# cristianpjensen/thesis-pai-reconstruction

Hardware: AMD Instinct MI355X
Metric: train images/sec (256x256, bs=64) Pix2Pix step (higher is better)
Workload: dtype bf16; 1 GPU; Pix2Pix generator+PatchGAN GAN step, 256x256x1 pairs, 64 images/GPU (BASELINE configs[1]); global_batch=64, per_gpu_batch=64, loss_type=gan, parallelism=dp1, grad_bucket_dtype=f32

## Files before the change

thesis-pai-reconstruction_amd/csrc/gg_thin.hip:

```cpp
#include <stdlib.h>

#include "common.h"

#ifndef THIN_ABL
#define THIN_ABL 0
#endif
typedef __attribute__((ext_vector_type(8))) __bf16 bf8_t;
typedef __attribute__((ext_vector_type(4))) __bf16 bf4_t;
typedef __attribute__((ext_vector_type(4))) float f4_t;
typedef __attribute__((ext_vector_type(8))) short s8_t;
typedef __attribute__((ext_vector_type(8))) unsigned short us8_t;

__device__ uint4 g_zero_line_thin[16];


__device__ __forceinline__ bf8_t relu8(bf8_t f) {
    s8_t x = __builtin_bit_cast(s8_t, f);
    const s8_t z = {0, 0, 0, 0, 0, 0, 0, 0};
    return __builtin_bit_cast(bf8_t, __builtin_elementwise_max(x, z));
}

template <int S>
__device__ __forceinline__ us8_t thin_gather8(__amdgpu_buffer_rsrc_t rs, int e0, int ix0, int TW, bool valid) {
    typedef __attribute__((ext_vector_type(4))) unsigned u4_t;
    const int base = ix0 & ~1, o = ix0 & 1;
    const bool neg = valid && e0 + base < 0;
    const unsigned vo = valid ? (neg ? 0u : (unsigned)(e0 + base) * 2u) : 0x80000000u;
    unsigned out[4];
    if (S == 2) {
        u4_t a = __builtin_amdgcn_raw_buffer_load_b128(rs, (int)vo, 0, 0);
        u4_t b = __builtin_amdgcn_raw_buffer_load_b128(rs, (int)vo + 16, 0, 0);
        if (__builtin_amdgcn_ballot_w64(neg) != 0) {
            if (neg) { b = (u4_t){a[3], b[0], b[1], b[2]}; a = (u4_t){0u, a[0], a[1], a[2]}; }
        }
        const unsigned sel = o ? 0x07060302u : 0x05040100u;
        out[0] = __builtin_amdgcn_perm(a[1], a[0], sel);
        out[1] = __builtin_amdgcn_perm(a[3], a[2], sel);
        out[2] = __builtin_amdgcn_perm(b[1], b[0], sel);
        out[3] = __builtin_amdgcn_perm(b[3], b[2], sel);
    } else {
        u4_t a = __builtin_amdgcn_raw_buffer_load_b128(rs, (int)vo, 0, 0);
        unsigned a4 = __builtin_amdgcn_raw_buffer_load_b32(rs, (int)vo + 16, 0, 0);
        if (__builtin_amdgcn_ballot_w64(neg) != 0) {
            if (neg) { a4 = a[3]; a = (u4_t){0u, a[0], a[1], a[2]}; }
        }
        const unsigned sh = (unsigned)o * 16u;
        out[0] = __builtin_amdgcn_alignbit(a[1], a[0], sh);
        out[1] = __builtin_amdgcn_alignbit(a[2], a[1], sh);
        out[2] = __builtin_amdgcn_alignbit(a[3], a[2], sh);
        out[3] = __builtin_amdgcn_alignbit(a4, a[3], sh);
    }
    const bool edge = valid && (ix0 < 0 || ix0 + S * 7 >= TW);
    if (__builtin_amdgcn_ballot_w64(edge) != 0) {
#pragma unroll
        for (int i = 0; i < 4; ++i) {
            const bool lo = (unsigned)(ix0 + S * (2 * i)) < (unsigned)TW, hi = (unsigned)(ix0 + S * (2 * i + 1)) < (unsigned)TW;
            out[i] &= (lo ? 0xffffu : 0u) | (hi ? 0xffff0000u : 0u);
        }
    }
    us8_t r;
#pragma unroll
    for (int i = 0; i < 4; ++i) { r[2 * i] = (unsigned short)(out[i] & 0xffffu); r[2 * i + 1] = (unsigned short)(out[i] >> 16); }
    return r;
}

__device__ __forceinline__ unsigned relu2u(unsigned v) {
    typedef __attribute__((ext_vector_type(2))) short s2_t;
    const s2_t z = {0, 0};
    return __builtin_bit_cast(unsigned, __builtin_elementwise_max(__builtin_bit_cast(s2_t, v), z));
}

__device__ __forceinline__ uint2 thin_gather4(__amdgpu_buffer_rsrc_t rs, int e0, int ix0, int TW, bool valid) {
    typedef __attribute__((ext_vector_type(3))) unsigned u3_t;
    const int base = ix0 & ~1, o = ix0 & 1;
    const bool neg = valid && e0 + base < 0;
    const unsigned vo = valid ? (neg ? 0u : (unsigned)(e0 + base) * 2u) : 0x80000000u;
    u3_t a = __builtin_amdgcn_raw_buffer_load_b96(rs, (int)vo, 0, 0);
    if (__builtin_amdgcn_ballot_w64(neg) != 0) {
        if (neg) a = (u3_t){0u, a[0], a[1]};
    }
    const unsigned sh = (unsigned)o * 16u;
    uint2 out = make_uint2(__builtin_amdgcn_alignbit(a[1], a[0], sh), __builtin_amdgcn_alignbit(a[2], a[1], sh));
    const bool edge = valid && (ix0 < 0 || ix0 + 3 >= TW);
    if (__builtin_amdgcn_ballot_w64(edge) != 0) {
        out.x &= ((unsigned)ix0 < (unsigned)TW ? 0xffffu : 0u) | ((unsigned)(ix0 + 1) < (unsigned)TW ? 0xffff0000u : 0u);
        out.y &= ((unsigned)(ix0 + 2) < (unsigned)TW ? 0xffffu : 0u) | ((unsigned)(ix0 + 3) < (unsigned)TW ? 0xffff0000u : 0u);
    }
    return out;
}

__device__ __forceinline__ void decode_row2(const GG& g, int m, int& n, int& gy, int& gx) {
    if (g.lw >= 0) {
        gx = m & (g.OWg - 1);
        gy = (m >> g.lw) & (g.OHg - 1);
        n = m >> (g.lw + g.lh);
    } else {
        gx = m % g.OWg;
        int r = m / g.OWg;
        gy = r % g.OHg;
        n = r / g.OHg;
    }
}

bool thin_fwd_ok(int dtype, const GG& g, const FwdArgs& a) {
    const bool taps_ok = g.ntaps == 16 || (g.ntaps == 9 && g.S == 1 && g.C2 == 0);
    return dtype == PAI_BF16 && g.nphase == 1 && taps_ok && g.OS == 1 && g.C1 == 1 && g.C2 <= 1 &&
           (g.Cout % 64) == 0 && g.Cout <= 128 && !a.stats && !a.yf32 && !a.skip_d1 &&
           (g.D2 == 0 || (g.D1 % 16) == 0);
}

template <int T>
__global__ __launch_bounds__(256) void thin_fwd_k(GG g, FwdArgs a, int fast_ok) {
    const int tid = threadIdx.x, lane = tid & 63, wid = tid >> 6;
    const int fr = lane & 15, fq = lane >> 4;
    const bf16_t* x1 = (const bf16_t*)a.x1;
    const bf16_t* x2 = (const bf16_t*)a.x2;
    const bf16_t* w = (const bf16_t*)a.w;
    const int mtiles = g.Cout / 16;
    const int KT = g.ntaps * T;
    const bool sect = (fast_ok & 2) != 0;
    fast_ok &= 1;

    bf8_t af[8];
#pragma unroll
    for (int mt = 0; mt < 8; ++mt) {
        us8_t z = {0, 0, 0, 0, 0, 0, 0, 0};
        const int co = sect ? 64 * (mt >> 2) + 32 * ((mt & 3) >> 1) + 8 * (fr >> 2) + 4 * (mt & 1) + (fr & 3)
                            : 64 * (mt >> 2) + 16 * (fr >> 2) + 4 * (mt & 3) + (fr & 3);
        if (mt < mtiles) {
            if ((KT & 7) == 0) {
                if (8 * fq < KT) z = *(const us8_t*)(w + (size_t)co * KT + 8 * fq);
            } else {
#pragma unroll
                for (int e = 0; e < 8; ++e)
                    if (8 * fq + e < KT) z[e] = w[(size_t)co * KT + 8 * fq + e];
            }
        }
        af[mt] = __builtin_bit_cast(bf8_t, z);
    }
    float bias[2][16];
#pragma unroll
    for (int gq = 0; gq < 2; ++gq)
#pragma unroll
        for (int e = 0; e < 16; ++e)
            bias[gq][e] = (a.bias && gq * 4 < mtiles) ? a.bias[64 * gq + (sect ? 32 * (e >> 3) + 8 * fq + (e & 7) : 16 * fq + e)] : 0.f;
    int pdy[8], pdx[8];
// ... 597 lines not shown
        const int hy0 = (oyl >> 1) + 1, hx0 = (oxl >> 1) + 1;
        const size_t o = ((size_t)n * g.OH + oy) * g.OW + ox;
#pragma unroll
        for (int tt = 0; tt < T; ++tt) {
            const int t = t0 + tt;
            float v = a.bias ? a.bias[t] : 0.f;
#pragma unroll
            for (int k = 0; k < 4; ++k) {
                const int e = tab[ph][k];
                const int hy = hy0 + (int)(signed char)(e & 0xff), hx = hx0 + (int)(signed char)((e >> 8) & 0xff);
                v += Ys[tt][hy * TU_HW + hx][(e >> 16) & 0xff];
            }
            if (t < g.D1) {
                if (a.y1 && !a.skip_d1) ((bf16_t*)a.y1)[o * g.D1 + t] = f2bf(v);
            } else if (a.y2) {
                ((bf16_t*)a.y2)[o * g.D2 + (t - g.D1)] = f2bf(v);
            }
            if (a.yact || a.yf32) {
                const float av = act_apply(v, a.eact);
                if (a.yact) ((bf16_t*)a.yact)[o * g.Cout + t] = f2bf(av);
                if (a.yf32) a.yf32[o * g.Cout + t] = av;
            }
        }
    }
}

static bool thin_up_ok(const GG& g) {
    return pai_tunable("thin_up", 1) && g.nphase == 4 && g.ntaps == 4 && g.OS == 2 && g.wtaps == 16 && (g.H % 16) == 0 &&
           (g.W % 16) == 0 && (g.Cin == 64 || g.Cin == 128);
}

int launch_thin_dgrad(const GG& g, const FwdArgs& a, hipStream_t s) {
    const int T = thin_dgrad_T(g, a);
    const int t0 = (g.Cout == 2 && a.skip_d1) ? 1 : 0;
    if (thin_up_ok(g)) {
        const int tx = g.W / 16, ty = g.H / 16;
        const dim3 grid(g.N * tx * ty);
        if (T == 1 && g.Cin == 128) PAI_LAUNCH((thin_up_k<1, 4>), grid, dim3(256), 0, s, g, a, t0, tx, ty);
        else if (T == 1) PAI_LAUNCH((thin_up_k<1, 2>), grid, dim3(256), 0, s, g, a, t0, tx, ty);
        else if (g.Cin == 128) PAI_LAUNCH((thin_up_k<2, 4>), grid, dim3(256), 0, s, g, a, t0, tx, ty);
        else PAI_LAUNCH((thin_up_k<2, 2>), grid, dim3(256), 0, s, g, a, t0, tx, ty);
        PAI_LAUNCH_CHECK();
        return 0;
    }
    int blocks = cdiv((int64_t)g.N * g.H * g.W, 256);
    if (blocks > 4096) blocks = 4096;
#define TDG(TT, KK) PAI_LAUNCH((thin_dgrad_gemm_k<TT, KK>), dim3(blocks), dim3(256), 0, s, g, a, pai_ctx()->scratch, t0)
#define TDG_K(TT)                                     \
    switch (g.Cin / 32) {                             \
        case 1: TDG(TT, 1); break;                    \
        case 2: TDG(TT, 2); break;                    \
        case 4: TDG(TT, 4); break;                    \
        case 8: TDG(TT, 8); break;                    \
        case 16: TDG(TT, 16); break;                  \
        default: PAI_CHECK(false, "thin dgrad: unsupported Cin %d", g.Cin); \
    }
    if (T == 1) { TDG_K(1) } else { TDG_K(2) }
#undef TDG_K
#undef TDG
    PAI_LAUNCH_CHECK();
    PAI_CHECK((int64_t)g.N * g.OH * g.OW < (1ll << 31), "thin dgrad: more than 2^31 output pixels");
    int64_t b2 = ((int64_t)g.N * g.OH * g.OW + 255) / 256;
    if (b2 > 8192) b2 = 8192;
    PAI_LAUNCH(thin_col2im_k, dim3((int)b2), dim3(256), 0, s, g, a, (const float*)pai_ctx()->scratch, T, t0);
    PAI_LAUNCH_CHECK();
    return 0;
}

struct ThinW {
    const bf16_t *thin1, *thin2;
    const bf16_t *wide1, *wide2;
    int N, H, W, TH, TW, WC1, WC2;
    int relu1, relu2;
    int lw, lh;
    int tmul, flip;
    int kw, ntaps;
    float* dw;
    int s_wc, s_tap, s_t;
    float* dbias;
    int M;
    int fast;
    int pair;
    float* partial;
};

__device__ __forceinline__ int tw_swz(int row) { return ((row & 3) << 2) | ((row >> 2) & 3); }
__device__ __forceinline__ unsigned tw_off(int row, int ch) { return (unsigned)(256 * row + 16 * (ch ^ tw_swz(row))); }

#ifndef THIN_WG_WAVES
#define THIN_WG_WAVES 1
#endif
template <int T>
__global__ __launch_bounds__(256, THIN_WG_WAVES) void thin_wgrad_k(ThinW p, int chunks_per_block) {
    extern __shared__ __attribute__((aligned(16))) unsigned char smem[];
    const int tid = threadIdx.x, lane = tid & 63;
    const int wid = __builtin_amdgcn_readfirstlane(tid >> 6);
    const int fr = lane & 15, fq = lane >> 4, tq = fr >> 2, tp = fr & 3;
    const int wc0 = blockIdx.y * 128;
    const int WC = min(p.WC1 + p.WC2 - wc0, 128);
    const int pair = p.pair;
    const int ntile = pair ? 8 : WC / 16;
    const int ks = wid & 1;
    const int nt0 = (wid >> 1) * (ntile / 2);
    const int ntn = ntile / 2;
    const int pixh = pair ? (wid >> 1) * 64 : 0;
    const int CH = pair ? 128 : 64;
    const bf16_t* zero = (const bf16_t*)g_zero_line_thin;

    const int sc = lane & 15, sr = wid * 4 + (lane >> 4);
    const int gch = sc ^ tw_swz(sr);
    const bf16_t* wsrc;
    int wstride, wcol;
    bool wvalid = pair || gch * 8 < WC;
    const int wpix = pair ? (gch >> 3) * 64 : 0;
    if (pair) { wsrc = p.wide1; wstride = p.WC1; wcol = (gch & 7) * 8; }
    else if (wc0 + gch * 8 < p.WC1) { wsrc = p.wide1; wstride = p.WC1; wcol = wc0 + gch * 8; }
    else { wsrc = p.wide2; wstride = p.WC2; wcol = gch * 8 - p.WC1; }

    int kdy[T], kdx[T];
    const bf16_t* ksrc[T];
    int kt[T];
#pragma unroll
    for (int tt = 0; tt < T; ++tt) {
        const int k = 16 * tt + fr;
        const int tap = k / T, t = k - tap * T;
        const int th = tap / p.kw, tw = tap - th * p.kw;
        kdy[tt] = p.flip ? 1 - th : th - 1;
        kdx[tt] = tap < p.ntaps ? (p.flip ? 1 - tw : tw - 1) : -(1 << 20);
        ksrc[tt] = t ? p.thin2 : p.thin1;
        kt[tt] = t;
    }
    const unsigned thin_bytes = (unsigned)(p.N * p.TH * p.TW) * 2u;
    const __amdgpu_buffer_rsrc_t trs1 = __builtin_amdgcn_make_buffer_rsrc(const_cast<bf16_t*>(p.thin1), 0, thin_bytes, 0x00020000);
    const __amdgpu_buffer_rsrc_t trs2 = __builtin_amdgcn_make_buffer_rsrc(
        const_cast<bf16_t*>(p.thin2 ? p.thin2 : p.thin1), 0, p.thin2 ? thin_bytes : 0u, 0x00020000);

    f4_t acc[T][4];
#pragma unroll
    for (int tt = 0; tt < T; ++tt)
#pragma unroll
        for (int j = 0; j < 4; ++j) acc[tt][j] = (f4_t){0.f, 0.f, 0.f, 0.f};
    f4_t accb[4];
#pragma unroll
    for (int j = 0; j < 4; ++j) accb[j] = (f4_t){0.f, 0.f, 0.f, 0.f};
    const unsigned one2 = fr == 0 ? 0x3f803f80u : 0u;
    const bf8_t ones = __builtin_bit_cast(bf8_t, make_uint4(one2, one2, one2, one2));

    for (int ci = 0; ci < chunks_per_block; ++ci) {
        const int p0 = (blockIdx.x * chunks_per_block + ci) * CH;
        if (p0 >= p.M) break;
#pragma unroll
        for (int j = 0; j < 4; ++j) {
            const int m = p0 + wpix + sr + 16 * j;
            const bf16_t* src = (wvalid && m < p.M) ? wsrc + (size_t)m * wstride + wcol : zero;
            __builtin_amdgcn_global_load_lds((const __attribute__((address_space(1))) void*)src,
                                             (__attribute__((address_space(3))) void*)(smem + (16 * j + wid * 4) * 256),
                                             16, 0, 0);
        }
        bf8_t af[T];
#pragma unroll
        for (int tt = 0; tt < T; ++tt) {
            us8_t pv;
            if (p.fast) {
                const int m = p0 + pixh + 32 * ks + 8 * fq;
                int n, ay, bx;
                if (p.lw >= 0) { bx = m & (p.W - 1); ay = (m >> p.lw) & (p.H - 1); n = m >> (p.lw + p.lh); }
                else { bx = m % p.W; const int r = m / p.W; ay = r % p.H; n = r / p.H; }
                const int iy = p.tmul * ay + kdy[tt], ix0 = p.tmul * bx + kdx[tt];
                const bool rowok = m < p.M && (unsigned)iy < (unsigned)p.TH && kdx[tt] > -(1 << 19);
                const int e0 = (n * p.TH + iy) * p.TW;
                if (p.tmul == 2) pv = kt[tt] ? thin_gather8<2>(trs2, e0, ix0, p.TW, rowok) : thin_gather8<2>(trs1, e0, ix0, p.TW, rowok);
                else pv = kt[tt] ? thin_gather8<1>(trs2, e0, ix0, p.TW, rowok) : thin_gather8<1>(trs1, e0, ix0, p.TW, rowok);
            } else {
#pragma unroll
            for (int j = 0; j < 8; ++j) {
                const int m = p0 + pixh + 32 * ks + 8 * fq + j;
                int n, ay, bx;
                if (p.lw >= 0) { bx = m & (p.W - 1); ay = (m >> p.lw) & (p.H - 1); n = m >> (p.lw + p.lh); }
                else { bx = m % p.W; const int r = m / p.W; ay = r % p.H; n = r / p.H; }
                const int iy = p.tmul * ay + kdy[tt], ix = p.tmul * bx + kdx[tt];
                const bool inb = m < p.M && (unsigned)iy < (unsigned)p.TH && (unsigned)ix < (unsigned)p.TW;
                pv[j] = inb ? ksrc[tt][(size_t)(n * p.TH + iy) * p.TW + ix] : (unsigned short)0;
            }
            }
            af[tt] = __builtin_bit_cast(bf8_t, pv);
        }
        __syncthreads();
#pragma unroll
        for (int nt = 0; nt < 4; ++nt) {
            if (nt >= ntn) break;
            const int col0 = (nt0 + nt) * 16;
            bf8_t bfr;
#pragma unroll
            for (int h = 0; h < 2; ++h) {
                const int row = ks * 32 + fq * 8 + h * 4 + tq;
                const int ch = col0 / 8 + (tp >> 1);
                bf4_t v = __builtin_amdgcn_ds_read_tr16_b64_v4bf16(
                    (bf4_t __attribute__((address_space(3)))*)(smem + tw_off(row, ch) + 8 * (tp & 1)));
#pragma unroll
                for (int e = 0; e < 4; ++e) bfr[h * 4 + e] = v[e];
            }
            if ((pair || wc0 + col0 < p.WC1) ? p.relu1 : p.relu2) bfr = relu8(bfr);
#pragma unroll
            for (int tt = 0; tt < T; ++tt)
                acc[tt][nt] = __builtin_amdgcn_mfma_f32_16x16x32_bf16(af[tt], bfr, acc[tt][nt], 0, 0, 0);
            if (p.dbias) accb[nt] = __builtin_amdgcn_mfma_f32_16x16x32_bf16(ones, bfr, accb[nt], 0, 0, 0);
        }
        __syncthreads();
    }
    float* part0 = p.partial ? p.partial + (((size_t)blockIdx.x * 2) * gridDim.y + blockIdx.y) * ((16 * T + 1) * 128) : nullptr;
    float* part = part0 ? part0 + (size_t)ks * gridDim.y * ((16 * T + 1) * 128) : nullptr;
#pragma unroll
    for (int tt = 0; tt < T; ++tt)
#pragma unroll
        for (int nt = 0; nt < 4; ++nt) {
            if (nt >= ntn) break;
            const int wcl = (nt0 + nt) * 16 + fr;
#pragma unroll
            for (int r = 0; r < 4; ++r) {
                const int k = 16 * tt + 4 * fq + r;
                if (part) {
                    part[k * 128 + wcl] = acc[tt][nt][r];
                } else {
                    const int tap = k / T, t = k - tap * T;
                    if (tap < p.ntaps)
                        atomicAdd(p.dw + (size_t)(wc0 + (pair ? (wcl & 63) : wcl)) * p.s_wc + tap * p.s_tap + t * p.s_t, acc[tt][nt][r]);
                }
            }
        }
    if (p.dbias) {
        float* red = (float*)smem;
        __syncthreads();
        if (fq == 0) {
#pragma unroll
            for (int nt = 0; nt < 4; ++nt)
                if (nt < ntn) red[ks * 128 + (nt0 + nt) * 16 + fr] = accb[nt][0];
        }
        __syncthreads();
        if (tid < (pair ? 128 : WC)) {
            if (part0) {
                part0[16 * T * 128 + tid] = red[tid] + red[tid + 128];
                part0[(size_t)gridDim.y * ((16 * T + 1) * 128) + 16 * T * 128 + tid] = 0.f;
            } else {
                atomicAdd(p.dbias + wc0 + (pair ? (tid & 63) : tid), red[tid] + red[tid + 128]);
            }
        }
    }
}

__global__ __launch_bounds__(256) void thin_wgrad_reduce_k(ThinW p, int T, int ntiles, int groups) {
    __shared__ float red[4][64];
    const int pst = (16 * T + 1) * 128;
    const int e = blockIdx.x * 64 + (threadIdx.x & 63), slice = threadIdx.x >> 6;
    const int gy = e / pst, le = e - gy * pst;
    const int per = (ntiles + gridDim.y - 1) / gridDim.y;
    const int b0 = blockIdx.y * per, b1 = min(ntiles, b0 + per);
    float sum = 0.f;
    if (gy < groups) {
        const float* src = p.partial + (size_t)gy * pst + le;
        const size_t bstride = (size_t)groups * pst;
        int b = b0 + slice;
        for (; b + 28 < b1; b += 32) {
            float t[8];
#pragma unroll
            for (int u = 0; u < 8; ++u) t[u] = src[(size_t)(b + 4 * u) * bstride];
            sum += ((t[0] + t[1]) + (t[2] + t[3])) + ((t[4] + t[5]) + (t[6] + t[7]));
        }
        for (; b < b1; b += 4) sum += src[(size_t)b * bstride];
    }
    red[slice][threadIdx.x & 63] = sum;
    __syncthreads();
    if (slice == 0 && gy < groups) {
        sum = red[0][threadIdx.x] + red[1][threadIdx.x] + red[2][threadIdx.x] + red[3][threadIdx.x];
        const int k = le >> 7;
        int wc = gy * 128 + (le & 127);
        if (p.pair) wc &= 63;
        if (wc < p.WC1 + p.WC2) {
            if (k < 16 * T) {
                const int tap = k / T, t = k - tap * T;
                if (tap < p.ntaps) atomicAdd(p.dw + (size_t)wc * p.s_wc + tap * p.s_tap + t * p.s_t, sum);
            } else if (p.dbias) {
                atomicAdd(p.dbias + wc, sum);
            }
        }
    }
}

__global__ __launch_bounds__(256) void sum1_k(const bf16_t* x, int64_t n, float* out) {
    __shared__ float ws[4];
    float s = 0.f;
    const int64_t n8 = n >> 3;
    for (int64_t i = (int64_t)blockIdx.x * 256 + threadIdx.x; i < n8; i += (int64_t)gridDim.x * 256) {
        const uint4 v = ((const uint4*)x)[i];
        const unsigned w4[4] = {v.x, v.y, v.z, v.w};
#pragma unroll
        for (int e = 0; e < 4; ++e) s += __uint_as_float(w4[e] << 16) + __uint_as_float(w4[e] & 0xffff0000u);
    }
    for (int64_t i = n8 * 8 + (int64_t)blockIdx.x * 256 + threadIdx.x; i < n; i += (int64_t)gridDim.x * 256) s += bf2f(x[i]);
    s = wave_sum(s);
    if ((threadIdx.x & 63) == 0) ws[threadIdx.x >> 6] = s;
    __syncthreads();
    if (threadIdx.x == 0) atomicAdd(out, ws[0] + ws[1] + ws[2] + ws[3]);
}

static int ilog2_exact(int v) {
    int l = 0;
    while ((1 << l) < v) ++l;
    return (1 << l) == v ? l : -1;
}

bool thin_wgrad_conv_ok(int dtype, const GG& g) {
    return dtype == PAI_BF16 && g.nphase == 1 && g.ntaps == 16 && g.S == 2 && g.OS == 1 && g.C1 == 1 &&
           g.C2 <= 1 && (g.Cout % 32) == 0 && g.Cout <= 128 && !g.relu1 && !g.relu2;
}
bool thin_wgrad_convt_ok(int dtype, const GG& g) {
    return dtype == PAI_BF16 && g.nphase == 4 && g.ntaps == 4 && g.Cout == 1 && (g.C1 % 8) == 0 &&
           (g.C2 % 8) == 0 && (g.Cin % 32) == 0 && g.Cin <= 128;
}

static int tw_blocks(int64_t M, int groups, bool two_stage) {
    static const int cap_env = getenv("PAI_TW_BLOCKS") ? atoi(getenv("PAI_TW_BLOCKS")) : 0;
    int cap = cap_env ? cap_env : (two_stage ? 1024 / groups : 512);
    if (cap < 64) cap = 64;
    const int chunks = cdiv(M, 64);
    int blocks = chunks < cap ? chunks : cap;
    const int cpb = cdiv(chunks, blocks);
    return cdiv(chunks, cpb);
}

int64_t thin_wgrad_scratch_bytes(int64_t M, int T, int WC) {
    return (int64_t)tw_blocks(M, cdiv(WC, 128), true) * 2 * cdiv(WC, 128) * (16 * T + 1) * 128 * sizeof(float);
}

static int launch_tw(ThinW& p, int T, hipStream_t s) {
    p.M = p.N * p.H * p.W;
    p.fast = pai_tunable("thin_fast", 1) && (p.W % 8) == 0 && (p.TW % 2) == 0 && (p.tmul == 1 || p.tmul == 2) &&
             (int64_t)p.N * p.TH * p.TW * 2 < (1ll << 31);
    p.lw = ilog2_exact(p.W);
    p.lh = ilog2_exact(p.H);
    if (p.lw < 0 || p.lh < 0) p.lw = p.lh = -1;
    p.pair = pai_tunable("thin_pair", 1) && p.WC1 == 64 && p.WC2 == 0 && T == 2;
    const int chunks = cdiv(p.M, p.pair ? 128 : 64);
    const int groups = cdiv(p.WC1 + p.WC2, 128);
    const int64_t need = thin_wgrad_scratch_bytes(p.M, T, p.WC1 + p.WC2);
    static const bool no_two = getenv("PAI_TW_ATOMIC") && atoi(getenv("PAI_TW_ATOMIC")) != 0;
    const pai_handle_s* ctx = pai_ctx();
    const bool two_stage = !no_two && ctx->scratch != nullptr && ctx->scratch_bytes >= need;
    int blocks = tw_blocks(p.M, groups, two_stage);
    const int cpb = cdiv(chunks, blocks);
    p.partial = two_stage ? (float*)((char*)ctx->scratch + (ctx->scratch_bytes - need)) : nullptr;
    if (T == 1) PAI_LAUNCH(thin_wgrad_k<1>, dim3(blocks, groups), dim3(256), 64 * 256, s, p, cpb);
    else PAI_LAUNCH(thin_wgrad_k<2>, dim3(blocks, groups), dim3(256), 64 * 256, s, p, cpb);
    PAI_LAUNCH_CHECK();
    if (two_stage) {
        const int elems = groups * (16 * T + 1) * 128;
        PAI_LAUNCH(thin_wgrad_reduce_k, dim3(cdiv(elems, 64), 16), dim3(256), 0, s, p, T, blocks * 2, groups);
        PAI_LAUNCH_CHECK();
    }
    return 0;
}

int launch_thin_wgrad_conv(const GG& g, const WgradArgs& a, hipStream_t s) {
    ThinW p;
    memset(&p, 0, sizeof(p));
    const int T = g.C1 + g.C2;
    p.thin1 = (const bf16_t*)a.x1; p.thin2 = (const bf16_t*)a.x2;
    p.wide1 = (const bf16_t*)a.dy; p.wide2 = nullptr;
    p.N = g.N; p.H = g.OHg; p.W = g.OWg; p.TH = g.H; p.TW = g.W;
    p.WC1 = g.Cout; p.WC2 = 0;
    p.dw = a.dw; p.s_wc = 16 * T; p.s_tap = T; p.s_t = 1;
    p.dbias = a.dbias;
    p.tmul = 2; p.flip = 0; p.kw = 4; p.ntaps = 16;
    return launch_tw(p, T, s);
}

int launch_thin_wgrad_convt(const GG& g, const WgradArgs& a, hipStream_t s) {
    ThinW p;
    memset(&p, 0, sizeof(p));
    p.thin1 = (const bf16_t*)a.dy; p.thin2 = nullptr;
    p.wide1 = (const bf16_t*)a.x1; p.wide2 = (const bf16_t*)a.x2;
    p.N = g.N; p.H = g.H; p.W = g.W; p.TH = g.OH; p.TW = g.OW;
    p.WC1 = g.C1; p.WC2 = g.C2; p.relu1 = g.relu1; p.relu2 = g.relu2;
    p.dw = a.dw; p.s_wc = 1; p.s_tap = g.Cin; p.s_t = 0;
    p.dbias = nullptr;
    p.tmul = 2; p.flip = 0; p.kw = 4; p.ntaps = 16;
    if (launch_tw(p, 1, s)) return 1;
    if (a.dbias) {
        const int64_t n = (int64_t)g.N * g.OH * g.OW;
        PAI_LAUNCH(sum1_k, dim3(256), dim3(256), 0, s, (const bf16_t*)a.dy, n, a.dbias);
        PAI_LAUNCH_CHECK();
    }
    return 0;
}

bool thin_wgrad_conv1_ok(int dtype, const GG& g) {
    return dtype == PAI_BF16 && g.nphase == 1 && g.ntaps == 16 && g.S == 1 && g.OS == 1 && g.Cout == 1 &&
           g.C2 == 0 && (g.C1 % 128) == 0;
}

int launch_thin_wgrad_conv1(const GG& g, const WgradArgs& a, hipStream_t s) {
    ThinW p;
    memset(&p, 0, sizeof(p));
    p.thin1 = (const bf16_t*)a.dy; p.thin2 = nullptr;
    p.wide1 = (const bf16_t*)a.x1; p.wide2 = nullptr;
    p.N = g.N; p.H = g.H; p.W = g.W; p.TH = g.OH; p.TW = g.OW;
    p.WC1 = g.C1; p.WC2 = 0; p.relu1 = g.relu1;
    p.dw = a.dw; p.s_wc = 1; p.s_tap = g.Cin; p.s_t = 0;
    p.dbias = nullptr;
    p.tmul = 1; p.flip = 1; p.kw = 4; p.ntaps = 16;
    if (launch_tw(p, 1, s)) return 1;
    if (a.dbias) {
        const int64_t n = (int64_t)g.N * g.OH * g.OW;
        PAI_LAUNCH(sum1_k, dim3(64), dim3(256), 0, s, (const bf16_t*)a.dy, n, a.dbias);
        PAI_LAUNCH_CHECK();
    }
    return 0;
}

bool thin_wgrad_conv3_ok(int dtype, const GG& g) {
    return dtype == PAI_BF16 && g.nphase == 1 && g.ntaps == 9 && g.S == 1 && g.OS == 1 && g.C1 == 1 && g.C2 == 0 &&
           (g.Cout % 32) == 0 && g.Cout <= 128 && !g.relu1;
}

int launch_thin_wgrad_conv3(const GG& g, const WgradArgs& a, hipStream_t s) {
    ThinW p;
    memset(&p, 0, sizeof(p));
    p.thin1 = (const bf16_t*)a.x1; p.thin2 = nullptr;
    p.wide1 = (const bf16_t*)a.dy; p.wide2 = nullptr;
    p.N = g.N; p.H = g.OHg; p.W = g.OWg; p.TH = g.H; p.TW = g.W;
    p.WC1 = g.Cout; p.WC2 = 0;
    p.dw = a.dw; p.s_wc = 9; p.s_tap = 1; p.s_t = 0;
    p.dbias = a.dbias;
    p.tmul = 1; p.flip = 0; p.kw = 3; p.ntaps = 9;
    return launch_tw(p, 1, s);
}

bool thin_wgrad_conv3t_ok(int dtype, const GG& g) {
    return dtype == PAI_BF16 && g.nphase == 1 && g.ntaps == 9 && g.S == 1 && g.OS == 1 && g.Cout == 1 && g.C2 == 0 &&
           (g.C1 % 32) == 0 && g.C1 <= 128;
// ... 21 lines not shown
```

thesis-pai-reconstruction_amd/csrc/gg_wg3.hip:

```cpp
#include <type_traits>

#include "gg_tile.h"

__device__ __forceinline__ int tr_swz3(int row) { return ((row & 3) << 2) | ((row >> 2) & 3); }
__device__ __forceinline__ unsigned tr_off3(int row, int ch) { return (unsigned)(256 * row + 16 * (ch ^ tr_swz3(row))); }
template <int CI, int BW> __device__ __forceinline__ unsigned xseg_swz3(unsigned p) {
    if (BW == 8) return ((p >> 1) & 1u) | (((p >> 2) & 1u) << 1);
    return CI == 64 ? (((p >> 1) & 1u) | (((p >> 3) & 1u) << 1)) : ((p & 3u) | (((p >> 3) & 1u) << 2));
}
template <int BMC> __device__ __forceinline__ int yswz3(int row) {
    return BMC == 128 ? tr_swz3(row) : ((((row >> 1) & 1) | (((row >> 3) & 1) << 1)) << 1);
}

#ifndef WG3_PRIO
#define WG3_PRIO 0
#endif
#ifndef WG3_SPREAD
#define WG3_SPREAD 0
#endif
#ifndef WG3_ADDR
#define WG3_ADDR 1
#endif
#ifndef WG3_ABL
#define WG3_ABL 0
// ... 570 lines not shown
    const size_t rstep = (size_t)g.wtaps * g.Cin;
    auto store_tile = [&](auto mode_tag) {
        constexpr int MODE = decltype(mode_tag)::value;
#pragma unroll
        for (int mt = 0; mt < MT; ++mt)
#pragma unroll
            for (int r = 0; r < 4; ++r) {
                float* prow = pw0 + (size_t)(mt * 16 + r) * rstep;
#pragma unroll
                for (int nt = 0; nt < NT; ++nt) {
                    float* pw = prow + nt * 16;
                    if (WG3_ABL & 1) { if (acc[mt][nt][r] == 123.456f) *pw = 0.f; }
                    else if (MODE == 0) *pw = acc[mt][nt][r];
                    else if (MODE == 1) *pw += acc[mt][nt][r];
                    else atomicAdd(pw, acc[mt][nt][r]);
                }
            }
    };
    if (a.slab || (splits == 1 && a.overwrite)) store_tile(std::integral_constant<int, 0>{});
    else if (splits == 1) store_tile(std::integral_constant<int, 1>{});
    else store_tile(std::integral_constant<int, 2>{});
}

__global__ __launch_bounds__(256) void wgrad_slab_sum_k(float* __restrict__ dw, const float* __restrict__ slab, int nsplits,
                                                        long n4, long slab_stride4, int overwrite) {
    __shared__ float4 red[3][64];
    const int e = threadIdx.x & 63, q = threadIdx.x >> 6;
    const long i = (long)blockIdx.x * 64 + e;
    float4 v = make_float4(0.f, 0.f, 0.f, 0.f);
    if (i < n4) {
        const float4* s = (const float4*)slab + i;
        int k = q;
        for (; k + 28 < nsplits; k += 32) {
            float4 t[8];
#pragma unroll
            for (int u = 0; u < 8; ++u) t[u] = s[(long)(k + 4 * u) * slab_stride4];
#pragma unroll
            for (int u = 0; u < 8; ++u) { v.x += t[u].x; v.y += t[u].y; v.z += t[u].z; v.w += t[u].w; }
        }
        for (; k < nsplits; k += 4) {
            const float4 t = s[(long)k * slab_stride4];
            v.x += t.x; v.y += t.y; v.z += t.z; v.w += t.w;
        }
    }
    if (q) red[q - 1][e] = v;
    __syncthreads();
    if (q == 0 && i < n4) {
#pragma unroll
        for (int j = 0; j < 3; ++j) { v.x += red[j][e].x; v.y += red[j][e].y; v.z += red[j][e].z; v.w += red[j][e].w; }
        if (!overwrite) {
            const float4 o = ((const float4*)dw)[i];
            v.x += o.x; v.y += o.y; v.z += o.z; v.w += o.w;
        }
        ((float4*)dw)[i] = v;
    }
}

template <int NS>
__global__ __launch_bounds__(256) void wgrad_slab_sum_few_k(float* __restrict__ dw, const float* __restrict__ slab, long n4,
                                                            long slab_stride4, int overwrite) {
    constexpr int U = 4;
    const long stride = (long)gridDim.x * 256;
    for (long i0 = (long)blockIdx.x * 256 + threadIdx.x; i0 < n4; i0 += stride * U) {
        float4 t[U][NS], o[U];
#pragma unroll
        for (int u = 0; u < U; ++u) {
            const long i = i0 + u * stride;
#pragma unroll
            for (int k = 0; k < NS; ++k) t[u][k] = i < n4 ? ((const float4*)slab)[(long)k * slab_stride4 + i] : make_float4(0.f, 0.f, 0.f, 0.f);
            if (!overwrite) o[u] = i < n4 ? ((const float4*)dw)[i] : make_float4(0.f, 0.f, 0.f, 0.f);
        }
#pragma unroll
        for (int u = 0; u < U; ++u) {
            const long i = i0 + u * stride;
            float4 v = t[u][0];
#pragma unroll
            for (int k = 1; k < NS; ++k) { v.x += t[u][k].x; v.y += t[u][k].y; v.z += t[u][k].z; v.w += t[u][k].w; }
            if (!overwrite) { v.x += o[u].x; v.y += o[u].y; v.z += o[u].z; v.w += o[u].w; }
            if (i < n4) ((float4*)dw)[i] = v;
        }
    }
}

int launch_wgrad_slab_sum(float* dw, const float* slab, int nsplits, int64_t n, int overwrite, hipStream_t s) {
    PAI_CHECK((n % 4) == 0, "wgrad slab sum: %lld elements are not a multiple of 4", (long long)n);
    const long n4 = (long)(n / 4);
    if (nsplits >= 2 && nsplits <= 4 && pai_tunable("slab_sum_few", 1)) {
        long blocks = (n4 + 256 * 4 - 1) / (256 * 4);
        if (blocks > 2048) blocks = 2048;
        if (nsplits == 2) PAI_LAUNCH(wgrad_slab_sum_few_k<2>, dim3((unsigned)blocks), dim3(256), 0, s, dw, slab, n4, n4, overwrite);
        else if (nsplits == 3) PAI_LAUNCH(wgrad_slab_sum_few_k<3>, dim3((unsigned)blocks), dim3(256), 0, s, dw, slab, n4, n4, overwrite);
        else PAI_LAUNCH(wgrad_slab_sum_few_k<4>, dim3((unsigned)blocks), dim3(256), 0, s, dw, slab, n4, n4, overwrite);
        PAI_LAUNCH_CHECK();
        return 0;
    }
    PAI_LAUNCH(wgrad_slab_sum_k, dim3((unsigned)((n4 + 63) / 64)), dim3(256), 0, s, dw, slab, nsplits, n4, n4, overwrite);
    PAI_LAUNCH_CHECK();
    return 0;
}

static int wg3_variant(const GG& g, PatchGeo* pg) {
    const int mode = pai_tunable("wgrad3", 7);
    if (!mode) return 0;
    if ((int64_t)g.N * g.H * g.W * (g.C1 > g.C2 ? g.C1 : g.C2) * 2 >= (1ll << 31) || (int64_t)g.N * g.OH * g.OW * g.Cout * 2 >= (1ll << 31))
        return 0;
    if (g.lsw >= 0 && g.lw == 3 && g.lh >= 3 && patch_geo(g, 8, pg, 8))
        return ((mode & 4) && (g.Cout % 128) == 0 && (g.C1 % 64) == 0 && (g.C2 % 64) == 0 && g.Cin >= 64) ? WG3_128x64_8 : 0;
    if (!(g.lsw >= 0 && g.lw >= 4 && g.lh >= 2 && patch_geo(g, 4, pg))) return 0;
    if ((g.Cout % 128) == 0 && (g.C1 % 64) == 0 && (g.C2 % 64) == 0 && g.Cin >= 64) return (mode & 1) ? WG3_128x64 : 0;
    if ((g.Cout % 64) == 0 && (g.C1 % 128) == 0 && (g.C2 % 128) == 0 && g.Cin >= 128) return (mode & 2) ? WG3_64x128 : 0;
    return 0;
}

bool wgrad3_ok(const GG& g) {
    PatchGeo pg;
    return wg3_variant(g, &pg) != 0;
}

static int wg3_psplits(const GG& g, int tiles, int solo, int* per) {
    const int kblocks = g.M / 64;
    int splits = cdiv(solo ? pai_tunable("wgrad3_target_solo", 512) : pai_tunable("wgrad3_target", 256), tiles);
    const int max_splits = cdiv(g.M, pai_tunable("wgrad3_minrows", 512));
    if (splits > max_splits) splits = max_splits;
    if (splits < 1) splits = 1;
    *per = cdiv(kblocks, splits);
    return cdiv(kblocks, *per);
}

MfmaPlan wgrad3_plan(const GG& g, bool has_dbias) {
    static const char* const names[3] = {"gg_wgrad_patch3_k<128, 64, 16>", "gg_wgrad_patch3_k<64, 128, 16>", "gg_wgrad_patch3_k<128, 64, 8>"};
    MfmaPlan p = {};
    const int v = wg3_variant(g, &p.pg);
    if (!v) return p;
    p.variant = v;
    p.name = names[v - WG3_128x64];
    p.bm = v == WG3_64x128 ? 64 : 128;
    p.bn = v == WG3_64x128 ? 128 : 64;
    p.mtiles = g.Cout / p.bm;
    p.ntiles = (g.Cin / p.bn) * p.pg.groups;
    const int tiles = p.mtiles * p.ntiles * g.nphase;
    p.ksplit = wg3_psplits(g, tiles, g.solo, &p.rows);
    int per;
    const int ps0 = wg3_psplits(g, tiles, 0, &per), ps1 = wg3_psplits(g, tiles, 1, &per), ps = ps0 > ps1 ? ps0 : ps1;
    const int64_t dw_bytes = (int64_t)g.Cout * g.wtaps * g.Cin * 4;
    p.workspace_bytes = ps > 1 ? ps * dw_bytes : 0;
    p.overwrites = p.ksplit == 1 || (pai_tunable("wgrad_slab", 1) && wgrad_slab_acquire(p.ksplit * dw_bytes) != nullptr);
    p.db = pai_tunable("wgrad3_pipe", 1) && !has_dbias;
    p.lds = (size_t)2 * (v == WG3_128x64 ? 64 * 256 + 96 * 128 : (v == WG3_64x128 ? 64 * 128 + 96 * 256 : 64 * 256 + 128 * 128));
    p.grid = tiles * p.ksplit;
    p.block = 256;
    return p;
}

int launch_wgrad3(const GG& g, const WgradArgs& a0, const MfmaPlan& p, hipStream_t s) {
    WgradArgs a = a0;
    const int64_t dwn = (int64_t)g.Cout * g.wtaps * g.Cin;
    float* slab = nullptr;
    if (p.ksplit > 1 && pai_tunable("wgrad_slab", 1)) slab = wgrad_slab_acquire((int64_t)p.ksplit * dwn * 4);
    a.slab = slab;
    if (a.overwrite_bias && a.dbias) {
        hipError_t e = pai::memset_async(a.dbias, 0, (size_t)g.Cout * sizeof(float), s);
        PAI_CHECK(e == hipSuccess, "launch_wgrad3: hipMemsetAsync: %s", hipGetErrorString(e));
    }
    static PerDeviceOnce attr;
    if (attr.first()) {
        hipError_t e = hipSuccess;
        const void* fns[6] = {reinterpret_cast<const void*>(&gg_wgrad_patch3_k<128, 64, 16>), reinterpret_cast<const void*>(&gg_wgrad_patch3_k<64, 128, 16>),
                              reinterpret_cast<const void*>(&gg_wgrad_patch3_k<128, 64, 8>), reinterpret_cast<const void*>(&gg_wgrad_patch3_k<128, 64, 16, 0>),
                              reinterpret_cast<const void*>(&gg_wgrad_patch3_k<64, 128, 16, 0>), reinterpret_cast<const void*>(&gg_wgrad_patch3_k<128, 64, 8, 0>)};
// ... 18 lines not shown
```

Before: 11380 images/s.

## Add software-pipelined per-wave thin wgrad kernel and wide slab-sum reducer

Adds a new thin-channel weight-gradient kernel in which each wave independently prefetches its next wide tile via global_load_lds and issues the next thin gathers while computing MFMAs on the current step. Gather is split into issue and finish halves so load latency overlaps compute. Cross-wave reduction goes through LDS and writes a tap-major partial layout, signalled to the reduce kernel by a new kperm flag. Separately adds a wide slab-sum kernel for five or more splits, which spreads splits across four waves and reduces them in LDS. The trade is more register and LDS use per wave, 32KB instead of 16KB of LDS per block, plus a more complex code path.

```diff
diff --git a/thesis-pai-reconstruction_amd/csrc/gg_thin.hip b/thesis-pai-reconstruction_amd/csrc/gg_thin.hip
--- a/thesis-pai-reconstruction_amd/csrc/gg_thin.hip
+++ b/thesis-pai-reconstruction_amd/csrc/gg_thin.hip
@@ -20,16 +20,28 @@
     return __builtin_bit_cast(bf8_t, __builtin_elementwise_max(x, z));
 }
 
+typedef __attribute__((ext_vector_type(4))) unsigned u4_t;
+struct ThinRaw { u4_t a, b; };
+
 template <int S>
-__device__ __forceinline__ us8_t thin_gather8(__amdgpu_buffer_rsrc_t rs, int e0, int ix0, int TW, bool valid) {
-    typedef __attribute__((ext_vector_type(4))) unsigned u4_t;
+__device__ __forceinline__ ThinRaw thin_gather8_issue(__amdgpu_buffer_rsrc_t rs, int e0, int ix0, bool valid) {
+    const int base = ix0 & ~1;
+    const bool neg = valid && e0 + base < 0;
+    const unsigned vo = valid ? (neg ? 0u : (unsigned)(e0 + base) * 2u) : 0x80000000u;
+    ThinRaw r;
+    r.a = __builtin_amdgcn_raw_buffer_load_b128(rs, (int)vo, 0, 0);
+    if (S == 2) r.b = __builtin_amdgcn_raw_buffer_load_b128(rs, (int)vo + 16, 0, 0);
+    else r.b = (u4_t){__builtin_amdgcn_raw_buffer_load_b32(rs, (int)vo + 16, 0, 0), 0u, 0u, 0u};
+    return r;
+}
+
+template <int S>
+__device__ __forceinline__ us8_t thin_gather8_finish(ThinRaw raw, int e0, int ix0, int TW, bool valid) {
     const int base = ix0 & ~1, o = ix0 & 1;
     const bool neg = valid && e0 + base < 0;
-    const unsigned vo = valid ? (neg ? 0u : (unsigned)(e0 + base) * 2u) : 0x80000000u;
     unsigned out[4];
     if (S == 2) {
-        u4_t a = __builtin_amdgcn_raw_buffer_load_b128(rs, (int)vo, 0, 0);
-        u4_t b = __builtin_amdgcn_raw_buffer_load_b128(rs, (int)vo + 16, 0, 0);
+        u4_t a = raw.a, b = raw.b;
         if (__builtin_amdgcn_ballot_w64(neg) != 0) {
             if (neg) { b = (u4_t){a[3], b[0], b[1], b[2]}; a = (u4_t){0u, a[0], a[1], a[2]}; }
         }
@@ -39,8 +51,8 @@
         out[2] = __builtin_amdgcn_perm(b[1], b[0], sel);
         out[3] = __builtin_amdgcn_perm(b[3], b[2], sel);
     } else {
-        u4_t a = __builtin_amdgcn_raw_buffer_load_b128(rs, (int)vo, 0, 0);
-        unsigned a4 = __builtin_amdgcn_raw_buffer_load_b32(rs, (int)vo + 16, 0, 0);
+        u4_t a = raw.a;
+        unsigned a4 = raw.b[0];
         if (__builtin_amdgcn_ballot_w64(neg) != 0) {
             if (neg) { a4 = a[3]; a = (u4_t){0u, a[0], a[1], a[2]}; }
         }
@@ -62,6 +74,11 @@
 #pragma unroll
     for (int i = 0; i < 4; ++i) { r[2 * i] = (unsigned short)(out[i] & 0xffffu); r[2 * i + 1] = (unsigned short)(out[i] >> 16); }
     return r;
+}
+
+template <int S>
+__device__ __forceinline__ us8_t thin_gather8(__amdgpu_buffer_rsrc_t rs, int e0, int ix0, int TW, bool valid) {
+    return thin_gather8_finish<S>(thin_gather8_issue<S>(rs, e0, ix0, valid), e0, ix0, TW, valid);
 }
 
 __device__ __forceinline__ unsigned relu2u(unsigned v) {
@@ -825,6 +842,7 @@
     int fast;
     int pair;
     float* partial;
+    int kperm;
 };
 
 __device__ __forceinline__ int tw_swz(int row) { return ((row & 3) << 2) | ((row >> 2) & 3); }
@@ -991,6 +1009,188 @@
     }
 }
 
+template <int T, bool PACK, int GATHER>
+__global__ __launch_bounds__(256) void thin_wgrad_wave_k(ThinW p, int steps_per_block) {
+    extern __shared__ __attribute__((aligned(16))) unsigned char smem[];
+    constexpr int P = PACK ? 64 : 32;
+    constexpr int NH = PACK ? 2 : 1;
+    constexpr int NACC = PACK ? 4 : 8;
+    const int tid = threadIdx.x, lane = tid & 63;
+    const int wid = __builtin_amdgcn_readfirstlane(tid >> 6);
+    const int fr = lane & 15, fq = lane >> 4, tq = fr >> 2, tp = fr & 3;
+    const int wc0 = blockIdx.y * 128;
+    const int WC = min(p.WC1 + p.WC2 - wc0, 128);
+    const int ntile = PACK ? 8 : WC / 16;
+    unsigned char* tile = smem + wid * (32 * 256);
+    const bf16_t* zero = (const bf16_t*)g_zero_line_thin;
+
+    const int sc = lane & 15, a4 = lane >> 4;
+    const bf16_t* wb[4];
+    int wst[4], wpx[4];
+#pragma unroll
+    for (int jj = 0; jj < 4; ++jj) {
+        const int gch = sc ^ ((a4 << 2) | jj);
+        wpx[jj] = 0;
+        if (PACK) { wb[jj] = p.wide1 + (gch & 7) * 8; wst[jj] = p.WC1; wpx[jj] = (gch >> 3) * 32; }
+        else if (gch * 8 >= WC) { wb[jj] = nullptr; wst[jj] = 0; }
+        else if (wc0 + gch * 8 < p.WC1) { wb[jj] = p.wide1 + wc0 + gch * 8; wst[jj] = p.WC1; }
+        else { wb[jj] = p.wide2 + (wc0 + gch * 8 - p.WC1); wst[jj] = p.WC2; }
+    }
+    auto fill = [&](int p0) {
+#pragma unroll
+        for (int j = 0; j < 8; ++j) {
+            const int m = p0 + wpx[j & 3] + 4 * j + a4;
+            const bf16_t* src = (wb[j & 3] && m < p.M) ? wb[j & 3] + (size_t)m * wst[j & 3] : zero;
+            __builtin_amdgcn_global_load_lds((const __attribute__((address_space(1))) void*)src,
+                                             (__attribute__((address_space(3))) void*)(tile + j * 1024), 16, 0, 0);
+        }
+    };
+
+    const int th = fr / p.kw, tw = fr - th * p.kw;
+    const int kdy = p.flip ? 1 - th : th - 1;
+    const int kdx = fr < p.ntaps ? (p.flip ? 1 - tw : tw - 1) : -(1 << 20);
+    const unsigned thin_bytes = (unsigned)(p.N * p.TH * p.TW) * 2u;
+    const __amdgpu_buffer_rsrc_t trs1 = __builtin_amdgcn_make_buffer_rsrc(const_cast<bf16_t*>(p.thin1), 0, thin_bytes, 0x00020000);
+    const __amdgpu_buffer_rsrc_t trs2 = __builtin_amdgcn_make_buffer_rsrc(
+        const_cast<bf16_t*>(p.thin2 ? p.thin2 : p.thin1), 0, p.thin2 ? thin_bytes : 0u, 0x00020000);
+    auto patch_at = [&](int m, int& e0, int& ix0, bool& rowok) {
+        int n, ay, bx;
+        if (GATHER || p.lw >= 0) { bx = m & (p.W - 1); ay = (m >> p.lw) & (p.H - 1); n = m >> (p.lw + p.lh); }
+        else { bx = m % p.W; const int r = m / p.W; ay = r % p.H; n = r / p.H; }
+        const int iy = p.tmul * ay + kdy;
+        ix0 = p.tmul * bx + kdx;
+        rowok = m < p.M && (unsigned)iy < (unsigned)p.TH && kdx > -(1 << 19);
+        e0 = (n * p.TH + iy) * p.TW;
+    };
+    ThinRaw raw[NH][T];
+    auto gather = [&](int p0) {
+#pragma unroll
+        for (int h = 0; h < NH; ++h) {
+            const int m0 = p0 + 32 * h + 8 * fq;
+            if (GATHER) {
+                int e0, ix0;
+                bool rowok;
+                patch_at(m0, e0, ix0, rowok);
+#pragma unroll
+                for (int tt = 0; tt < T; ++tt) raw[h][tt] = thin_gather8_issue<GATHER ? GATHER : 1>(tt ? trs2 : trs1, e0, ix0, rowok);
+            } else {
+                us8_t pv[T];
+#pragma unroll
+                for (int j = 0; j < 8; ++j) {
+                    int e0, ix;
+                    bool rowok;
+                    patch_at(m0 + j, e0, ix, rowok);
+                    const bool inb = rowok && (unsigned)ix < (unsigned)p.TW;
+#pragma unroll
+                    for (int tt = 0; tt < T; ++tt) pv[tt][j] = inb ? (tt ? p.thin2 : p.thin1)[(size_t)e0 + ix] : (unsigned short)0;
+                }
+#pragma unroll
+                for (int tt = 0; tt < T; ++tt) raw[h][tt].a = __builtin_bit_cast(u4_t, pv[tt]);
+            }
+        }
+    };
+
+    f4_t acc[T][NACC], accb[NACC];
+#pragma unroll
+    for (int j = 0; j < NACC; ++j) {
+#pragma unroll
+        for (int tt = 0; tt < T; ++tt) acc[tt][j] = (f4_t){0.f, 0.f, 0.f, 0.f};
+        accb[j] = (f4_t){0.f, 0.f, 0.f, 0.f};
+    }
+    const unsigned one2 = fr == 0 ? 0x3f803f80u : 0u;
+    const bf8_t ones = __builtin_bit_cast(bf8_t, make_uint4(one2, one2, one2, one2));
+
+    const int step = 4 * P;
+    const long pend_l = (long)(blockIdx.x + 1) * steps_per_block * step;
+    const int pend = pend_l < p.M ? (int)pend_l : p.M;
+    int p0 = blockIdx.x * steps_per_block * step + wid * P;
+    if (p0 < pend) { fill(p0); gather(p0); }
+    for (; p0 < pend; p0 += step) {
+        __builtin_amdgcn_s_waitcnt(0x0f70);
+        __builtin_amdgcn_sched_barrier(0);
+        bf8_t af[NH][T];
+#pragma unroll
+        for (int h = 0; h < NH; ++h) {
+            int e0 = 0, ix0 = 0;
+            bool rowok = false;
+            if (GATHER) patch_at(p0 + 32 * h + 8 * fq, e0, ix0, rowok);
+#pragma unroll
+            for (int tt = 0; tt < T; ++tt) {
+                if (GATHER) af[h][tt] = __builtin_bit_cast(bf8_t, thin_gather8_finish<GATHER ? GATHER : 1>(raw[h][tt], e0, ix0, p.TW, rowok));
+                else af[h][tt] = __builtin_bit_cast(bf8_t, raw[h][tt].a);
+            }
+        }
+        bf8_t bfr[8];
+#pragma unroll
+        for (int nt = 0; nt < 8; ++nt) {
+            if (nt >= ntile) break;
+#pragma unroll
+            for (int h = 0; h < 2; ++h) {
+                const int row = fq * 8 + h * 4 + tq;
+                const int ch = nt * 2 + (tp >> 1);
+                bf4_t v = __builtin_amdgcn_ds_read_tr16_b64_v4bf16(
+                    (bf4_t __attribute__((address_space(3)))*)(tile + tw_off(row, ch) + 8 * (tp & 1)));
+#pragma unroll
+                for (int e = 0; e < 4; ++e) bfr[nt][h * 4 + e] = v[e];
+            }
+        }
+        __builtin_amdgcn_s_waitcnt(0xc07f);
+        __builtin_amdgcn_sched_barrier(0);
+        if (p0 + step < pend) { fill(p0 + step); gather(p0 + step); }
+        __builtin_amdgcn_sched_barrier(0);
+#pragma unroll
+        for (int nt = 0; nt < 8; ++nt) {
+            if (nt >= ntile) break;
+            const int ai = PACK ? (nt & 3) : nt, h = PACK ? (nt >> 2) : 0;
+            bf8_t b = bfr[nt];
+            if ((PACK || wc0 + ai * 16 < p.WC1) ? p.relu1 : p.relu2) b = relu8(b);
+#pragma unroll
+            for (int tt = 0; tt < T; ++tt)
+                acc[tt][ai] = __builtin_amdgcn_mfma_f32_16x16x32_bf16(af[h][tt], b, acc[tt][ai], 0, 0, 0);
+            if (p.dbias) accb[ai] = __builtin_amdgcn_mfma_f32_16x16x32_bf16(ones, b, accb[ai], 0, 0, 0);
+        }
+    }
+    const int ncols = PACK ? 64 : WC;
+    float* red = (float*)smem;
+    __syncthreads();
+    for (int w = 0; w < 4; ++w) {
+        if (wid == w) {
+#pragma unroll
+            for (int ai = 0; ai < NACC; ++ai) {
+                if (ai * 16 >= ncols) break;
+                const int col = ai * 16 + fr;
+#pragma unroll
+                for (int tt = 0; tt < T; ++tt)
+#pragma unroll
+                    for (int r = 0; r < 4; ++r) {
+                        float* d = red + (16 * tt + 4 * fq + r) * 128 + col;
+                        *d = w ? *d + acc[tt][ai][r] : acc[tt][ai][r];
+                    }
+                if (p.dbias && fq == 0) {
+                    float* d = red + 16 * T * 128 + col;
+                    *d = w ? *d + accb[ai][0] : accb[ai][0];
+                }
+            }
+        }
+        __syncthreads();
+    }
+    float* part = p.partial ? p.partial + ((size_t)blockIdx.x * gridDim.y + blockIdx.y) * ((16 * T + 1) * 128) : nullptr;
+    const int nel = (16 * T + (p.dbias ? 1 : 0)) * 128;
+    for (int el = tid; el < nel; el += 256) {
+        const int k = el >> 7, col = el & 127;
+        if (col >= ncols) continue;
+        const float v = red[el];
+        if (part) {
+            part[el] = v;
+        } else if (k < 16 * T) {
+            const int tap = k & 15, t = k >> 4;
+            if (tap < p.ntaps) atomicAdd(p.dw + (size_t)(wc0 + col) * p.s_wc + tap * p.s_tap + t * p.s_t, v);
+        } else {
+            atomicAdd(p.dbias + wc0 + col, v);
+        }
+    }
+}
+
 __global__ __launch_bounds__(256) void thin_wgrad_reduce_k(ThinW p, int T, int ntiles, int groups) {
     __shared__ float red[4][64];
     const int pst = (16 * T + 1) * 128;
@@ -1020,7 +1220,7 @@
         if (p.pair) wc &= 63;
         if (wc < p.WC1 + p.WC2) {
             if (k < 16 * T) {
-                const int tap = k / T, t = k - tap * T;
+                const int tap = p.kperm ? (k & 15) : k / T, t = p.kperm ? (k >> 4) : k - tap * T;
                 if (tap < p.ntaps) atomicAdd(p.dw + (size_t)wc * p.s_wc + tap * p.s_tap + t * p.s_t, sum);
             } else if (p.dbias) {
                 atomicAdd(p.dbias + wc, sum);
@@ -1061,18 +1261,17 @@
            (g.C2 % 8) == 0 && (g.Cin % 32) == 0 && g.Cin <= 128;
 }
 
-static int tw_blocks(int64_t M, int groups, bool two_stage) {
+static int tw_blocks(int chunks, int groups, bool two_stage) {
     static const int cap_env = getenv("PAI_TW_BLOCKS") ? atoi(getenv("PAI_TW_BLOCKS")) : 0;
     int cap = cap_env ? cap_env : (two_stage ? 1024 / groups : 512);
     if (cap < 64) cap = 64;
-    const int chunks = cdiv(M, 64);
     int blocks = chunks < cap ? chunks : cap;
     const int cpb = cdiv(chunks, blocks);
     return cdiv(chunks, cpb);
 }
 
 int64_t thin_wgrad_scratch_bytes(int64_t M, int T, int WC) {
-    return (int64_t)tw_blocks(M, cdiv(WC, 128), true) * 2 * cdiv(WC, 128) * (16 * T + 1) * 128 * sizeof(float);
+    return (int64_t)tw_blocks((int)cdiv(M, 64), cdiv(WC, 128), true) * 2 * cdiv(WC, 128) * (16 * T + 1) * 128 * sizeof(float);
 }
 
 static int launch_tw(ThinW& p, int T, hipStream_t s) {
@@ -1082,22 +1281,43 @@
     p.lw = ilog2_exact(p.W);
     p.lh = ilog2_exact(p.H);
     if (p.lw < 0 || p.lh < 0) p.lw = p.lh = -1;
-    p.pair = pai_tunable("thin_pair", 1) && p.WC1 == 64 && p.WC2 == 0 && T == 2;
-    const int chunks = cdiv(p.M, p.pair ? 128 : 64);
+    const int pipe = pai_tunable("thin_wgrad_pipe", 1) && (!p.fast || p.lw >= 0);
+    p.pair = pai_tunable("thin_pair", 1) && p.WC1 == 64 && p.WC2 == 0 && (T == 2 || pipe);
     const int groups = cdiv(p.WC1 + p.WC2, 128);
     const int64_t need = thin_wgrad_scratch_bytes(p.M, T, p.WC1 + p.WC2);
     static const bool no_two = getenv("PAI_TW_ATOMIC") && atoi(getenv("PAI_TW_ATOMIC")) != 0;
     const pai_handle_s* ctx = pai_ctx();
     const bool two_stage = !no_two && ctx->scratch != nullptr && ctx->scratch_bytes >= need;
-    int blocks = tw_blocks(p.M, groups, two_stage);
+    p.partial = two_stage ? (float*)((char*)ctx->scratch + (ctx->scratch_bytes - need)) : nullptr;
+    const int chunks = cdiv(p.M, pipe ? (p.pair ? 256 : 128) : (p.pair ? 128 : 64));
+    const int blocks = tw_blocks(chunks, groups, two_stage);
     const int cpb = cdiv(chunks, blocks);
-    p.partial = two_stage ? (float*)((char*)ctx->scratch + (ctx->scratch_bytes - need)) : nullptr;
-    if (T == 1) PAI_LAUNCH(thin_wgrad_k<1>, dim3(blocks, groups), dim3(256), 64 * 256, s, p, cpb);
-    else PAI_LAUNCH(thin_wgrad_k<2>, dim3(blocks, groups), dim3(256), 64 * 256, s, p, cpb);
+    int ntiles = blocks * 2;
+    if (pipe) {
+        ntiles = blocks;
+        const int gm = p.fast ? p.tmul : 0;
+#define TW_WAVE(T_, PACK_)                                                                                                       \
+    do {                                                                                                                         \
+        if (gm == 2) PAI_LAUNCH((thin_wgrad_wave_k<T_, PACK_, 2>), dim3(blocks, groups), dim3(256), 128 * 256, s, p, cpb);      \
+        else if (gm == 1) PAI_LAUNCH((thin_wgrad_wave_k<T_, PACK_, 1>), dim3(blocks, groups), dim3(256), 128 * 256, s, p, cpb); \
+        else PAI_LAUNCH((thin_wgrad_wave_k<T_, PACK_, 0>), dim3(blocks, groups), dim3(256), 128 * 256, s, p, cpb);              \
+    } while (0)
+        if (T == 1 && p.pair) TW_WAVE(1, true);
+        else if (T == 1) TW_WAVE(1, false);
+        else if (p.pair) TW_WAVE(2, true);
+        else TW_WAVE(2, false);
+#undef TW_WAVE
+        p.pair = 0;
+        p.kperm = 1;
+    } else if (T == 1) {
+        PAI_LAUNCH(thin_wgrad_k<1>, dim3(blocks, groups), dim3(256), 64 * 256, s, p, cpb);
+    } else {
+        PAI_LAUNCH(thin_wgrad_k<2>, dim3(blocks, groups), dim3(256), 64 * 256, s, p, cpb);
+    }
     PAI_LAUNCH_CHECK();
     if (two_stage) {
         const int elems = groups * (16 * T + 1) * 128;
-        PAI_LAUNCH(thin_wgrad_reduce_k, dim3(cdiv(elems, 64), 16), dim3(256), 0, s, p, T, blocks * 2, groups);
+        PAI_LAUNCH(thin_wgrad_reduce_k, dim3(cdiv(elems, 64), 16), dim3(256), 0, s, p, T, ntiles, groups);
         PAI_LAUNCH_CHECK();
     }
     return 0;
diff --git a/thesis-pai-reconstruction_amd/csrc/gg_wg3.hip b/thesis-pai-reconstruction_amd/csrc/gg_wg3.hip
--- a/thesis-pai-reconstruction_amd/csrc/gg_wg3.hip
+++ b/thesis-pai-reconstruction_amd/csrc/gg_wg3.hip
@@ -676,9 +676,88 @@
     }
 }
 
+template <int U>
+__global__ __launch_bounds__(256) void wgrad_slab_sum_wide_k(float* __restrict__ dw, const float* __restrict__ slab, int nsplits,
+                                                             long n4, long slab_stride4, int overwrite) {
+    constexpr int J = U > 2 ? 4 : 8;
+    __shared__ float4 red[3][U][64];
+    const int e = threadIdx.x & 63;
+    const int q = __builtin_amdgcn_readfirstlane(threadIdx.x >> 6);
+    const long i0 = (long)blockIdx.x * (64 * U) + e;
+    const float4* s[U];
+    float4 v[U];
+#pragma unroll
+    for (int u = 0; u < U; ++u) {
+        const long i = i0 + 64 * u;
+        s[u] = (const float4*)slab + (i < n4 ? i : n4 - 1);
+        v[u] = make_float4(0.f, 0.f, 0.f, 0.f);
+    }
+    int k = q;
+    for (; k + 4 * (J - 1) < nsplits; k += 4 * J) {
+        float4 t[U][J];
+#pragma unroll
+        for (int u = 0; u < U; ++u)
+#pragma unroll
+            for (int j = 0; j < J; ++j) t[u][j] = s[u][(long)(k + 4 * j) * slab_stride4];
+#pragma unroll
+        for (int u = 0; u < U; ++u)
+#pragma unroll
+            for (int j = 0; j < J; ++j) { v[u].x += t[u][j].x; v[u].y += t[u][j].y; v[u].z += t[u][j].z; v[u].w += t[u][j].w; }
+    }
+    const int left = k < nsplits ? (nsplits - k + 3) >> 2 : 0;
+    if (left) {
+        float4 t[U][J - 1];
+#pragma unroll
+        for (int j = 0; j < J - 1; ++j)
+            if (j < left) {
+#pragma unroll
+                for (int u = 0; u < U; ++u) t[u][j] = s[u][(long)(k + 4 * j) * slab_stride4];
+            }
+#pragma unroll
+        for (int j = 0; j < J - 1; ++j)
+            if (j < left) {
+#pragma unroll
+                for (int u = 0; u < U; ++u) { v[u].x += t[u][j].x; v[u].y += t[u][j].y; v[u].z += t[u][j].z; v[u].w += t[u][j].w; }
+            }
+    }
+    float4 o[U];
+    if (q == 0 && !overwrite) {
+#pragma unroll
+        for (int u = 0; u < U; ++u) { const long i = i0 + 64 * u; o[u] = ((const float4*)dw)[i < n4 ? i : n4 - 1]; }
+    }
+    if (q) {
+#pragma unroll
+        for (int u = 0; u < U; ++u) red[q - 1][u][e] = v[u];
+    }
+    __syncthreads();
+    if (q == 0) {
+#pragma unroll
+        for (int u = 0; u < U; ++u) {
+            const long i = i0 + 64 * u;
+#pragma unroll
+            for (int j = 0; j < 3; ++j) { const float4 r = red[j][u][e]; v[u].x += r.x; v[u].y += r.y; v[u].z += r.z; v[u].w += r.w; }
+            if (!overwrite) { v[u].x += o[u].x; v[u].y += o[u].y; v[u].z += o[u].z; v[u].w += o[u].w; }
+            if (i < n4) ((float4*)dw)[i] = v[u];
+        }
+    }
+}
+
 int launch_wgrad_slab_sum(float* dw, const float* slab, int nsplits, int64_t n, int overwrite, hipStream_t s) {
     PAI_CHECK((n % 4) == 0, "wgrad slab sum: %lld elements are not a multiple of 4", (long long)n);
     const long n4 = (long)(n / 4);
+    if (nsplits >= 5 && n4 > 0 && pai_tunable("slab_sum_wide", 1)) {
+        int U = pai_tunable("slab_sum_u", 0);
+        if (U < 1 || U > 4) U = n4 >= 131072 ? 4 : (n4 >= 65536 ? 2 : 1);
+        const unsigned blocks = (unsigned)((n4 + 64 * U - 1) / (64 * U));
+        switch (U) {
+            case 1: PAI_LAUNCH(wgrad_slab_sum_wide_k<1>, dim3(blocks), dim3(256), 0, s, dw, slab, nsplits, n4, n4, overwrite); break;
+            case 2: PAI_LAUNCH(wgrad_slab_sum_wide_k<2>, dim3(blocks), dim3(256), 0, s, dw, slab, nsplits, n4, n4, overwrite); break;
+            case 3: PAI_LAUNCH(wgrad_slab_sum_wide_k<3>, dim3(blocks), dim3(256), 0, s, dw, slab, nsplits, n4, n4, overwrite); break;
+            default: PAI_LAUNCH(wgrad_slab_sum_wide_k<4>, dim3(blocks), dim3(256), 0, s, dw, slab, nsplits, n4, n4, overwrite); break;
+        }
+        PAI_LAUNCH_CHECK();
+        return 0;
+    }
     if (nsplits >= 2 && nsplits <= 4 && pai_tunable("slab_sum_few", 1)) {
         long blocks = (n4 + 256 * 4 - 1) / (256 * 4);
         if (blocks > 2048) blocks = 2048;
```

Result: no change. 11460 images/s, median of 6 (+0.7%).
